# wzhe06/SparrowRecSys

Measured on AMD Instinct MI355X. Metric: ctr_samples_per_sec, higher is better.
Workload: dtype f32

## Files before the change

sparrowrecsys_amd/csrc/host_setup_v2.h:

```cpp
constexpr int V2_WAVES = 8;
struct V2Variant {
    int g_emb, kpc, h0c, h1c;
    size_t lds_bytes;
    void (*pack)(const V2Args, float*);
};
#define V2_LDS(G_EMB, DV, KPC, H0C, H1C, FOLD) \
    (sizeof(float) * (V2Lds<G_EMB, DV, KPC, H0C, H1C, FOLD>::total_pad + V2_WAVES * V2Lds<G_EMB, DV, KPC, H0C, H1C, FOLD>::stage_floats))
#define V2_VARIANT(G_EMB) {G_EMB, 1, 2, 1, V2_LDS(G_EMB, 4, 1, 2, 1, true), &k_v2_pack_image<G_EMB, 4, 1, 2, 1, true>}
const V2Variant kV2Variants[] = {
    V2_VARIANT(6),
    V2_VARIANT(4),
    V2_VARIANT(5), V2_VARIANT(3), V2_VARIANT(2),
};

struct V2JVariant {
    int g_big, njf, kpc;
    bool half;
    V2JKernel fn;
    V2JManyKernel fn_many;
};
#define V2J_VARIANT(G_BIG, NJF, HALF) \
    {G_BIG, NJF, 1, HALF, &k_deepfm_v2_joint<G_BIG, NJF, 1, 2, 1, V2_WAVES, HALF>, &k_deepfm_v2_joint_many<G_BIG, NJF, 1, 2, 1, V2_WAVES, HALF>}
#define V2J_BOTH(G_BIG, NJF) V2J_VARIANT(G_BIG, NJF, true), V2J_VARIANT(G_BIG, NJF, false)
const V2JVariant kV2JVariants[] = {
    V2J_BOTH(3, 3),
    V2J_BOTH(2, 2),
    V2J_BOTH(3, 2), V2J_BOTH(3, 1), V2J_BOTH(2, 3), V2J_BOTH(2, 1), V2J_BOTH(1, 3), V2J_BOTH(1, 2), V2J_BOTH(1, 1),
};

struct V2J1Variant { int g_big, njf; V2JKernel fn[2]; int image_floats; };
#define V2J1_VARIANT(G_BIG, NJF) \
    {G_BIG, NJF, {&k_deepfm_v2_joint1<G_BIG, NJF, false>, &k_deepfm_v2_joint1<G_BIG, NJF, true>}, V2J1Lds<G_BIG>::total_pad}
const V2J1Variant kV2J1Variants[] = {
    V2J1_VARIANT(3, 3), V2J1_VARIANT(2, 2), V2J1_VARIANT(3, 2), V2J1_VARIANT(3, 1), V2J1_VARIANT(2, 3), V2J1_VARIANT(2, 1),
    V2J1_VARIANT(1, 3), V2J1_VARIANT(1, 2), V2J1_VARIANT(1, 1),
};

bool match_v2_chain(sprk_engine* h) {
    const sprk_plan& p = h->plan;
    if (p.model_kind != SPRK_MODEL_DEEPFM_V2 || p.din.enabled || p.n_bufs != 2) return false;
    V2Args a;
    memset(&a, 0, sizeof(a));
    int g_emb = 0;
    while (g_emb < p.n_segs && p.segs[g_emb].kind == SPRK_SEG_ROWS) ++g_emb;
    if (g_emb < 1 || g_emb > V2_MAX_FIELDS) return false;
    if (p.n_id_cols > 8 || p.n_dense > 8 || p.n_dense < 1) return false;
    const int Dp = p.segs[0].row_stride;
    bool raw_over_4g = false;
    for (int g = 0; g < g_emb; ++g) {
        const sprk_seg& s = p.segs[g];
        if (s.row_stride != Dp || s.count * 4 != Dp || s.dst != g * Dp) return false;
        const size_t need = ((size_t)s.vocab + 1) * Dp * sizeof(float);
        if (h->slot_bytes[s.slot] < need) return false;
        if (need >= ((size_t)1 << 32)) raw_over_4g = true;
        a.emb_col[g] = s.field; a.emb_vocab[g] = s.vocab; a.table[g] = (const float*)h->slot_ptr[s.slot];
    }
    int si = g_emb;
    if (si >= p.n_segs || p.segs[si].kind != SPRK_SEG_DENSE || p.segs[si].field != 0 || p.segs[si].count > 8) return false;
    const int n_num = p.segs[si].count, num_off = p.segs[si].dst;
    ++si;
    if (si < p.n_segs && p.segs[si].kind == SPRK_SEG_ZERO) ++si;
// ... 62 lines not shown
        const V2Variant& vv = kV2Variants[v];
        if (!want_fold) continue;
        if (vv.g_emb == g_emb && vv.kpc == kpc && vv.h0c == h0c && vv.h1c == h1c) {
            V2Run run;
            memset(&run, 0, sizeof(run));
            size_t fo_floats = 0;
            for (int g = 0; g < g_emb; ++g) {
                int hit = -1;
                for (int i = 0; i < n_fo; ++i)
                    if (a.fo_col[i] == a.emb_col[g] && a.fo_vocab[i] == a.emb_vocab[g]) hit = i;
                if (hit < 0) return false;
                run.col[g] = a.emb_col[g]; run.vocab[g] = a.emb_vocab[g];
                run.table[g] = a.table[g];
                run.fo_off[g] = (unsigned)fo_floats;
                fo_floats += (size_t)a.emb_vocab[g] + 1;
            }
            if (fo_floats >= ((size_t)1 << 31)) return false;
            for (int g = 0; g < g_emb; ++g) {
                h->v2_w1_grp[g] = nullptr;
                for (int i = 0; i < n_fo; ++i)
                    if (a.fo_col[i] == a.emb_col[g] && a.fo_vocab[i] == a.emb_vocab[g]) h->v2_w1_grp[g] = a.w1[i];
            }
            run.F = a.F; run.ND = a.ND; run.n_num = a.n_num;
            run.h0w = a.h0w; run.fo_bias = a.fo_bias; run.head_bias = a.head_bias;
            h->v2run = run;
            h->v2 = a;
            h->v2_fo_floats = fo_floats;
            h->v2_variant = (int)v;
            h->rows_g_emb = g_emb;
            h->v2_rows_ok = kpc >= 1 && kpc <= 4 && h0c >= 1 && h1c >= 1 && !raw_over_4g;
            return true;
        }
    }
    if (kpc >= 1 && kpc <= 4 && h0c >= 1 && h1c >= 1 && !raw_over_4g) {
        h->v2 = a;
        h->rows_g_emb = g_emb;
        h->rows_from_v2 = true;
    }
    return false;
}

int setup_v2_joint(sprk_engine* h) {
    const V2Variant& vv = kV2Variants[h->v2_variant];
    if (vv.kpc != 1 || vv.h0c != 2 || vv.h1c != 1 || !h->tune.v2_joint) return SPRK_OK;
    const int KP = 16, H0 = 32, G = vv.g_emb;
    int big[V2_MAX_FIELDS], nbig = 0, jf[V2_MAX_FIELDS], njf = 0;
    for (int g = 0; g < G; ++g) {
        const long long v1 = (long long)h->v2run.vocab[g] + 1;
        if (v1 <= 32 && njf < V2J_MAX_JF) jf[njf++] = g;
        else big[nbig++] = g;
    }
    if (njf < 1 || nbig < 1 || nbig > 3) return SPRK_OK;
    bool half = h->tune.v2_half;
    float p_scale = 1.f, w_scale = 1.f;
    if (half) {
        std::vector<AbsmaxJob> rows_jobs;
        for (int b = 0; b < nbig; ++b) {
            const long long rows = (long long)h->v2run.vocab[big[b]] + 1;
            rows_jobs.push_back({h->v2_folded + (size_t)h->v2run.rowbase[big[b]] * (KP + 16), rows, KP + 16, KP, absmax_grid(rows * KP, 8192), 0});
        }
        SPRK_TRY(static_scale(rows_jobs, &p_scale));
        if (p_scale != 0.f) SPRK_TRY(static_scale({{h->v2.W0, (long long)H0, (G + 1) * KP, (G + 1) * KP, 8, 0}}, &w_scale));
        if (p_scale == 0.f || w_scale == 0.f) { half = false; p_scale = w_scale = 1.f; }
    }
    int variant = -1;
    for (size_t v = 0; v < sizeof(kV2JVariants) / sizeof(kV2JVariants[0]); ++v)
        if (kV2JVariants[v].g_big == nbig && kV2JVariants[v].njf == njf && kV2JVariants[v].half == half) variant = (int)v;
    if (variant < 0) return SPRK_OK;
    V2JRun& r = h->v2j_run;
    memset(&r, 0, sizeof(r));
    r.F = h->v2run.F; r.ND = h->v2run.ND; r.n_num = h->v2run.n_num;
    r.h0w = h->v2run.h0w; r.fo_bias = h->v2run.fo_bias; r.head_bias = h->v2run.head_bias;
    for (int b = 0; b < nbig; ++b) {
        r.big_col[b] = h->v2run.col[big[b]]; r.big_vocab[b] = h->v2run.vocab[big[b]];
        r.big_rowbase[b] = h->v2run.rowbase[big[b]]; r.big_grp[b] = big[b];
    }
    size_t small_floats = 0;
    for (int f = 0; f < njf; ++f) {
        r.j_col[f] = h->v2run.col[jf[f]]; r.j_vocab[f] = h->v2run.vocab[jf[f]];
        r.s_off[f] = (int)small_floats;
        small_floats += ((size_t)r.j_vocab[f] + 1) * V2J_SS;
    }
    small_floats = (small_floats + 255) & ~(size_t)255;
    r.wf_off = (int)small_floats;
    if (half) small_floats += ((size_t)H0 * 8 + 255) & ~(size_t)255;
    HIP_TRY(hipMalloc((void**)&h->v2j_tab, small_floats * sizeof(float)));
    HIP_TRY(hipMemset(h->v2j_tab, 0, small_floats * sizeof(float)));
    for (int f = 0; f < njf; ++f) {
        const int rows = r.j_vocab[f] + 1;
        hipLaunchKernelGGL(k_v2_fold_small, dim3((rows + 3) / 4), dim3(256), 0, 0,
                           h->v2_folded + (size_t)h->v2run.rowbase[jf[f]] * (KP + 16), KP, H0, jf[f], h->v2.W0, (G + 1) * KP,
                           h->v2.b0, f == 0 ? 1 : 0, h->v2j_tab + r.s_off[f], rows);
    }
    if (half)
        hipLaunchKernelGGL(k_v2j_fold_num, dim3(8), dim3(256), 0, 0, h->v2.W0, (G + 1) * KP, G * KP, h->v2.Wp[G], h->v2.ldp_num,
                           h->v2.bp[G], h->v2.n_num, KP, H0, h->v2j_tab + r.wf_off, h->v2j_tab + r.s_off[0], r.j_vocab[0] + 1);
    HIP_TRY(hipGetLastError());
    HIP_TRY(hipDeviceSynchronize());
    r.small_floats = (int)small_floats;
    r.tab0 = h->v2_folded;
    r.small = h->v2j_tab;
    r.w_scale = w_scale; r.unscale_h = 1.f / (p_scale * w_scale); r.unscale_s = 1.f / p_scale;
    if (half) {
        size_t big_rows = 0;
        for (int b = 0; b < nbig; ++b) big_rows += (size_t)r.big_vocab[b] + 1;
        if (big_rows * (KP + 16) * sizeof(float) >= ((size_t)1 << 32)) return fail(SPRK_EINVAL, "split rows exceed 32-bit offsets");
        SPRK_TRY(table_alloc(h, &h->v2j_big, big_rows * (KP + 16) * sizeof(float)));
        h->derived_bytes += big_rows * (KP + 16) * sizeof(float);
        size_t base = 0;
        for (int b = 0; b < nbig; ++b) {
            const long long rows = (long long)r.big_vocab[b] + 1;
            long long nb = (rows * 8 + 255) / 256;
            if (nb > 65536) nb = 65536;
            hipLaunchKernelGGL(k_v2_split_rows, dim3((unsigned)nb), dim3(256), 0, 0,
                               h->v2_folded + (size_t)r.big_rowbase[b] * (KP + 16), h->v2j_big + base * (KP + 16), rows, p_scale);
            r.big_rowbase[b] = (unsigned)base;
            base += (size_t)rows;
        }
        HIP_TRY(hipGetLastError());
        HIP_TRY(hipDeviceSynchronize());
        r.tab0 = h->v2j_big;
    }
    h->v2j_lds_bytes = vv.lds_bytes + small_floats * sizeof(float);
    SPRK_TRY(set_max_lds(kV2JVariants[variant].fn, h->v2j_lds_bytes));
    SPRK_TRY(set_max_lds(kV2JVariants[variant].fn_many, h->v2j_lds_bytes));
    h->v2j_variant = variant;
    if (half && h->tune.v2j_one) {
        for (size_t v = 0; v < sizeof(kV2J1Variants) / sizeof(kV2J1Variants[0]); ++v) {
            const V2J1Variant& ov = kV2J1Variants[v];
            if (ov.g_big != nbig || ov.njf != njf) continue;
            SPRK_TRY(dev_alloc(h, &h->v2j1_image, (size_t)ov.image_floats * sizeof(float)));
            hipLaunchKernelGGL(k_v2j1_pack_image, dim3(1), dim3(256), 0, 0, h->v2, r, nbig, G + 1, h->v2j1_image);
            HIP_TRY(hipGetLastError());
            HIP_TRY(hipDeviceSynchronize());
            const bool hoist = h->tune.v2j1_hoist >= 0 ? h->tune.v2j1_hoist != 0 : h->derived_bytes > ((size_t)256 << 20);
            h->v2j1_kernel = ov.fn[hoist];
            h->v2j1_waves = V2J1_WAVES_OF(hoist, nbig);
            h->v2j1_lds_bytes = ((size_t)ov.image_floats + small_floats + (size_t)h->v2j1_waves * 256) * sizeof(float);
            SPRK_TRY(set_max_lds(h->v2j1_kernel, h->v2j1_lds_bytes));
        }
    }
    return SPRK_OK;
}

int setup_v2_fold(sprk_engine* h) {
    const V2Variant& vv = kV2Variants[h->v2_variant];
    const int KP = vv.kpc * 16;
    h->v2_grid_cap = h->num_cus;
    SPRK_TRY(dev_alloc(h, &h->v2_fo_all, h->v2_fo_floats * sizeof(float)));
    for (int g = 0; g < vv.g_emb; ++g)
        HIP_TRY(hipMemcpy(h->v2_fo_all + h->v2run.fo_off[g], h->v2_w1_grp[g], ((size_t)h->v2run.vocab[g] + 1) * sizeof(float), hipMemcpyDeviceToDevice));
    h->v2run.fo_all = h->v2_fo_all;
    size_t rows_total = 0;
    for (int g = 0; g < vv.g_emb; ++g) { h->v2run.rowbase[g] = (unsigned)rows_total; rows_total += (size_t)h->v2run.vocab[g] + 1; }
    SPRK_TRY(table_alloc(h, &h->v2_folded, rows_total * (KP + 16) * sizeof(float)));
    for (int g = 0; g < vv.g_emb; ++g) {
        const long long rows = (long long)h->v2run.vocab[g] + 1;
        long long blocks = (rows + 3) / 4;
        if (blocks > 65536) blocks = 65536;
        hipLaunchKernelGGL(k_v2_fold, dim3((unsigned)blocks), dim3(256), 0, 0, h->v2.table[g], h->v2.ldp_emb,
                           h->v2.Wp[g], h->v2.ldp_emb, h->v2.bp[g], h->v2_w1_grp[g], h->v2.hfm, h->v2.n_hfm, h->v2.h0w,
                           h->v2_folded + (size_t)h->v2run.rowbase[g] * (KP + 16), KP, rows);
        HIP_TRY(hipGetLastError());
    }
    h->v2run.tab0 = h->v2_folded;
    HIP_TRY(hipDeviceSynchronize());
    SPRK_TRY(setup_v2_joint(h));
    if (h->v2j_variant < 0) {
        dev_free(h, h->v2_fo_all); h->v2_fo_all = nullptr;
        dev_free(h, h->v2_folded); h->v2_folded = nullptr;
        h->v2_variant = -1;
        h->rows_from_v2 = h->v2_rows_ok;
        return SPRK_OK;
    }
    h->derived_bytes += rows_total * (KP + 16) * sizeof(float);
    SPRK_TRY(dev_alloc(h, &h->v2_image, vv.lds_bytes));
    HIP_TRY(hipMemset(h->v2_image, 0, vv.lds_bytes));
    hipLaunchKernelGGL(vv.pack, dim3(1), dim3(256), 0, 0, h->v2, h->v2_image);
    HIP_TRY(hipGetLastError());
    HIP_TRY(hipDeviceSynchronize());
    return SPRK_OK;
}
```

sparrowrecsys_amd/csrc/k_chain_v2j.h:

```cpp

#define V2J_MAX_BIG 4
#define V2J_MAX_JF 3
#define V2J_SS 52

struct V2JRun {
    int F, ND, n_num;
    int big_col[V2J_MAX_BIG];
    int big_vocab[V2J_MAX_BIG];
    unsigned big_rowbase[V2J_MAX_BIG];
    int big_grp[V2J_MAX_BIG];
    int j_col[V2J_MAX_JF];
    int j_vocab[V2J_MAX_JF];
    int s_off[V2J_MAX_JF];
    int small_floats;
    int wf_off;
    const float* tab0;
    const float* small;
    float h0w, fo_bias, head_bias;
    int flags;
    float w_scale, unscale_h, unscale_s;
};

#define V2J_MB 64
struct V2JMany {
    const int* ids[V2J_MB];
    const float* dense[V2J_MB];
    float* out[V2J_MB];
    int n;
    int ntpb;
};

__device__ __forceinline__ void split_half4(f32x4 w, float scale, f16x4& hi, f16x4& lo) {
#pragma unroll
    for (int j = 0; j < 4; ++j) {
        const float x = w[j] * scale;
        const _Float16 h = (_Float16)x;
        hi[j] = h;
        lo[j] = (_Float16)(x - (float)h);
    }
}

static __global__ __launch_bounds__(256) void k_v2_absmax(const float* __restrict__ rows, long long nrows, int row_floats,
                                                   int ncols, unsigned* __restrict__ out) {
    float m = 0.f;
    const long long total = nrows * ncols;
    for (long long i = (long long)blockIdx.x * 256 + threadIdx.x; i < total; i += (long long)gridDim.x * 256) {
        const long long v = i / ncols;
        const int c = (int)(i - v * ncols);
        const float a = fabsf(rows[v * row_floats + c]);
        m = (a > m || a != a) ? a : m;
    }
    for (int d = 32; d >= 1; d >>= 1) { const float o = __shfl_xor(m, d); m = (o > m || o != o) ? o : m; }
    if ((threadIdx.x & 63) == 0) atomicMax(out, __float_as_uint(m));
}
static __global__ __launch_bounds__(256) void k_v2_count_small(const float* __restrict__ rows, long long nrows, int row_floats, int ncols,
                                                        float thresh, unsigned long long* __restrict__ out) {
    unsigned small = 0, nz = 0;
    const long long total = nrows * ncols;
    for (long long i = (long long)blockIdx.x * 256 + threadIdx.x; i < total; i += (long long)gridDim.x * 256) {
        const long long v = i / ncols;
        const int c = (int)(i - v * ncols);
        const float a = fabsf(rows[v * row_floats + c]);
        nz += a > 0.f;
        small += (a > 0.f && a < thresh);
    }
    for (int d = 32; d >= 1; d >>= 1) { small += __shfl_xor(small, d); nz += __shfl_xor(nz, d); }
    if ((threadIdx.x & 63) == 0) { atomicAdd(out, (unsigned long long)small); atomicAdd(out + 1, (unsigned long long)nz); }
}
static __global__ __launch_bounds__(256) void k_v2_split_rows(const float* __restrict__ src, float* __restrict__ dst,
                                                       long long nrows, float scale) {
    const long long total = nrows * 8;
    for (long long i = (long long)blockIdx.x * 256 + threadIdx.x; i < total; i += (long long)gridDim.x * 256) {
        const long long v = i >> 3;
// ... 11 lines not shown
}

static __global__ __launch_bounds__(256) void k_v2_fold_small(const float* __restrict__ folded, int KP, int H0, int grp,
                                                       const float* __restrict__ W0, int ldw0,
                                                       const float* __restrict__ b0, int add_b0,
                                                       float* __restrict__ out, int rows) {
    const int FS = KP + 16;
    for (int v = blockIdx.x * 4 + (threadIdx.x >> 6); v < rows; v += gridDim.x * 4) {
        const int col = threadIdx.x & 63;
        const float* prow = folded + (size_t)v * FS;
        float acc = 0.f;
        if (col < KP) {
            acc = prow[col];
        } else if (col < KP + H0) {
            const int m = col - KP;
            acc = add_b0 ? b0[m] : 0.f;
            const float* w = W0 + (size_t)m * ldw0 + grp * KP;
            for (int k = 0; k < KP; ++k) acc = fmaf(w[k], prow[k], acc);
        } else if (col == KP + H0) {
            acc = prow[KP];
        }
        if (col < V2J_SS) out[(size_t)v * V2J_SS + col] = acc;
    }
}

static __global__ __launch_bounds__(256) void k_v2j_fold_num(const float* __restrict__ W0, int ldw0, int num_off,
                                                      const float* __restrict__ Wn, int ldn, const float* __restrict__ bn,
                                                      int n_num, int KP, int H0, float* __restrict__ wf,
                                                      float* __restrict__ rows0, int nrows0) {
    for (int i = blockIdx.x * 256 + threadIdx.x; i < H0 * 8; i += gridDim.x * 256) {
        const int m = i >> 3, k = i & 7;
        double acc = 0.0;
        if (k < n_num)
            for (int n = 0; n < KP; ++n) acc += (double)W0[(size_t)m * ldw0 + num_off + n] * (double)Wn[(size_t)n * ldn + k];
        wf[i] = (float)acc;
    }
    for (int i = blockIdx.x * 256 + threadIdx.x; i < nrows0 * H0; i += gridDim.x * 256) {
        const int v = i / H0, m = i - v * H0;
        double acc = 0.0;
        for (int n = 0; n < KP; ++n) acc += (double)W0[(size_t)m * ldw0 + num_off + n] * (double)bn[n];
        rows0[(size_t)v * V2J_SS + KP + m] = (float)((double)rows0[(size_t)v * V2J_SS + KP + m] + acc);
    }
}

__device__ __forceinline__ f32x4 fma4s(f32x4 a, float b, f32x4 c) {
    return f32x4{__builtin_fmaf(a.x, b, c.x), __builtin_fmaf(a.y, b, c.y), __builtin_fmaf(a.z, b, c.z), __builtin_fmaf(a.w, b, c.w)};
}
__device__ __forceinline__ float dot4f(f32x4 a, f32x4 b) {
    return __builtin_fmaf(a.w, b.w, __builtin_fmaf(a.z, b.z, __builtin_fmaf(a.y, b.y, a.x * b.x)));
}
__device__ __forceinline__ f32x4 sq_diff4(f32x4 s, f32x4 p) {
    return f32x4{__builtin_fmaf(s.x, s.x, -(p.x * p.x)), __builtin_fmaf(s.y, s.y, -(p.y * p.y)), __builtin_fmaf(s.z, s.z, -(p.z * p.z)),
                 __builtin_fmaf(s.w, s.w, -(p.w * p.w))};
}

template <int G_BIG, int NJF>
struct V2JSet {
    f32x4 x[G_BIG];
    int so[NJF];
    f32x4 xn;
    float w1a;
};

template <int G_BIG, int NJF, int KPC, int H0C, int H1C, int WAVES, bool HALF, bool MB>
__device__ __forceinline__ void v2j_body(const V2JRun& A, const int* __restrict__ ids, const float* __restrict__ dense,
                                         float* __restrict__ out, int B, int* __restrict__ err,
                                         const float* __restrict__ image, const V2JMany* __restrict__ Mp) {
    constexpr int G_EMB = G_BIG + NJF;
    using LD = V2Lds<G_EMB, 4, KPC, H0C, H1C, true>;
    using Set = V2JSet<G_BIG, NJF>;
    constexpr int KP = LD::KP, H0 = H0C * 16;
    constexpr unsigned RB = (KP + 16) * 4;
    static_assert(KP + H0 + 1 <= V2J_SS, "small-field row layout");
    constexpr int NKR = HALF ? 1 : (G_BIG + 1) * KPC;
    static_assert(KPC == 1, "row layout: one 16-float chunk of projections per field");
    static_assert(G_BIG >= 1 && G_BIG <= 3 && NJF >= 1 && NJF <= V2J_MAX_JF, "field split");
    const int tid = threadIdx.x;
    const int lane = tid & 63;
    const int wave = __builtin_amdgcn_readfirstlane(tid >> 6);
    const int r = lane & 15, q = lane >> 4;
    const f32x4 zero = f32x4{0.f, 0.f, 0.f, 0.f};
    const int m_ntpb = MB ? Mp->ntpb : 0;
    const int ntasks = MB ? Mp->n * m_ntpb : (B + 15) >> 4;
    const int task_stride = gridDim.x * WAVES;
    const int wave_global = blockIdx.x * WAVES + wave;
    auto batch_of = [&](int tk, int& tl) {
        if constexpr (MB) {
            const int b = __builtin_amdgcn_readfirstlane(tk / m_ntpb);
            tl = tk - b * m_ntpb;
            return b;
        } else {
            tl = tk;
            return 0;
        }
    };
    float* stage = smem + LD::total_pad + wave * LD::stage_floats;
    const float* small_s = smem + LD::total_pad + WAVES * LD::stage_floats;
    const float* wq = smem + 4 * q;
    bool bad = false;
    const bool aligned = !(A.flags & 1);
    auto clampt = [&](int tk) { return tk < ntasks ? tk : ntasks - 1; };
    const int* const ids0 = ids;
    const float* const dense0 = dense;

    auto ld_raw = [&](int tkg, f32x4& raw) {
        int tk;
// ... 18 lines not shown
            const bool isid = lane < 32;
            const int j = isid ? lane : lane - 32;
            const int n4 = 4 * (isid ? A.F : A.ND);
            if (j < n4) st4(stage + (isid ? 0 : 128) + 4 * j, raw);
        } else {
            stage_task_slow(stage, ids, dense, A.F, A.ND, tk, B, lane);
        }
        const int* sid_row = reinterpret_cast<const int*>(stage) + r * A.F;
        unsigned sid[G_BIG];
#pragma unroll
        for (int b = 0; b < G_BIG; ++b) {
            const int id = sid_row[A.big_col[b]];
            bad |= (unsigned)(id + 1) > (unsigned)A.big_vocab[b];
            sid[b] = min((unsigned)id, (unsigned)A.big_vocab[b]) + A.big_rowbase[b];
        }
#pragma unroll
        for (int f = 0; f < NJF; ++f) {
            const int id = sid_row[A.j_col[f]];
            bad |= (unsigned)(id + 1) > (unsigned)A.j_vocab[f];
            S.so[f] = A.s_off[f] + (int)min((unsigned)id, (unsigned)A.j_vocab[f]) * V2J_SS;
        }
        {
            const float* nrow = stage + 128 + r * A.ND;
            const int c0 = 4 * q, last = A.n_num - 1;
            if constexpr (HALF) {
                S.xn.x = nrow[min(q, last)];
                S.xn.y = nrow[min(q + 4, last)];
            } else {
                S.xn.x = nrow[min(c0 + 0, last)];
                S.xn.y = nrow[min(c0 + 1, last)];
                S.xn.z = nrow[min(c0 + 2, last)];
                S.xn.w = nrow[min(c0 + 3, last)];
            }
        }
        const char* tb = reinterpret_cast<const char*>(A.tab0);
#pragma unroll
        for (int b = 0; b < G_BIG; ++b) S.x[b] = *reinterpret_cast<const f32x4*>(tb + (sid[b] * RB + 16u * q));
        {
            unsigned s0 = sid[0] * RB, s1 = sid[G_BIG > 1 ? 1 : 0] * RB, s2 = sid[G_BIG > 2 ? 2 : 0] * RB;
            asm("" : "+v"(s0), "+v"(s1), "+v"(s2));
            unsigned so = s0;
            if (G_BIG > 1) so = q == 1 ? s1 : so;
            if (G_BIG > 2) so = q == 2 ? s2 : so;
            S.w1a = *reinterpret_cast<const float*>(tb + (so + 4u * KP));
        }
    };

    f32x4 rW0[H0C][NKR], rW1[H1C][H0C];
    f32x4 rwn[KPC], rbpn[KPC], rb1[H1C], rhfm[KPC], rhd[H1C];
    f32x4 rfn = zero;
    float rwn8[2] = {0.f, 0.f}, rfn8[2] = {0.f, 0.f}, rwf[H0C][2];
    f16x8 hWa[HALF ? G_BIG : 1][H0C], hWb[HALF ? G_BIG : 1][H0C];
    f16x8 hSel = {0, 0, 0, 0, 0, 0, 0, 0};
    auto load_weights = [&]() {
        const float* w0r = wq + LD::off_w0 + r * LD::S0;
#pragma unroll
        for (int n0 = 0; n0 < H0C; ++n0) {
            if constexpr (HALF) {
                rwf[n0][0] = small_s[A.wf_off + (n0 * 16 + r) * 8 + q];
                rwf[n0][1] = small_s[A.wf_off + (n0 * 16 + r) * 8 + q + 4];
            } else {
                rW0[n0][0] = ld4(w0r + n0 * 16 * LD::S0 + 16 * G_EMB);
            }
#pragma unroll
            for (int b = 0; b < G_BIG; ++b) {
                const f32x4 w = ld4(w0r + n0 * 16 * LD::S0 + 16 * A.big_grp[b]);
                if constexpr (HALF) {
                    f16x4 hi, lo;
                    split_half4(w, A.w_scale, hi, lo);
                    hWa[b][n0] = f16x8{hi[0], hi[1], hi[2], hi[3], hi[0], hi[1], hi[2], hi[3]};
                    hWb[b][n0] = f16x8{lo[0], lo[1], lo[2], lo[3], lo[0], lo[1], lo[2], lo[3]};
                } else {
                    rW0[n0][(HALF ? 0 : 1 + b)] = w;
                }
            }
        }
        if constexpr (HALF) {
#pragma unroll
            for (int e = 0; e < 8; ++e) hSel[e] = (4 * q + (e & 3) == r) ? (_Float16)1.0f : (_Float16)0.0f;
        }
#pragma unroll
        for (int n1 = 0; n1 < H1C; ++n1) {
#pragma unroll
            for (int j = 0; j < H0C; ++j) rW1[n1][j] = ld4(wq + LD::off_w1 + (n1 * 16 + r) * LD::S1 + 16 * j);
            rb1[n1] = ld4(wq + LD::off_b1 + n1 * 16);
            rhd[n1] = ld4(wq + LD::off_hd + n1 * 16);
        }
#pragma unroll
        for (int nb = 0; nb < KPC; ++nb) {
            rwn[nb] = ld4(wq + LD::off_wn + (nb * 16 + r) * LD::SN);
            rbpn[nb] = ld4(wq + LD::off_bp + G_EMB * KP + nb * 16);
            rhfm[nb] = ld4(wq + LD::off_hfm + nb * 16);
        }
        rfn = ld4(smem + LD::off_fn + 4 * (q & 1));
        if constexpr (HALF) {
            rwn8[0] = smem[LD::off_wn + r * LD::SN + q];
            rwn8[1] = smem[LD::off_wn + r * LD::SN + q + 4];
            rfn8[0] = smem[LD::off_fn + q];
            rfn8[1] = smem[LD::off_fn + q + 4];
        }
    };

    auto compute = [&](const Set& S) -> float {
#pragma clang fp contract(off)
        const f32x4 pnum = S.xn;
        f32x4 pn;
        if constexpr (HALF) {
            const f32x4 e = __builtin_amdgcn_mfma_f32_16x16x4f32(rwn8[0], pnum.x, rbpn[0], 0, 0, 0);
            const f32x4 o = __builtin_amdgcn_mfma_f32_16x16x4f32(rwn8[1], pnum.y, zero, 0, 0, 0);
            pn = e + o;
        } else {
            f32x4 e = rbpn[0], o = zero;
            e = __builtin_amdgcn_mfma_f32_16x16x4f32(rwn[0].x, pnum.x, e, 0, 0, 0);
            o = __builtin_amdgcn_mfma_f32_16x16x4f32(rwn[0].y, pnum.y, o, 0, 0, 0);
            e = __builtin_amdgcn_mfma_f32_16x16x4f32(rwn[0].z, pnum.z, e, 0, 0, 0);
            o = __builtin_amdgcn_mfma_f32_16x16x4f32(rwn[0].w, pnum.w, o, 0, 0, 0);
            pn = e + o;
        }
        float zz = ((q < G_BIG) ? S.w1a : 0.f) + (HALF ? __builtin_fmaf(rfn8[1], pnum.y, rfn8[0] * pnum.x) : ((q < 2) ? dot4f(rfn, pnum) : 0.f));
        f32x4 sp = ld4(small_s + S.so[0] + 4 * q), sq[H0C];
#pragma unroll
        for (int n0 = 0; n0 < H0C; ++n0) sq[n0] = ld4(small_s + S.so[0] + KP + 16 * n0 + 4 * q);
        float ssc = small_s[S.so[0] + KP + H0];
#pragma unroll
        for (int f = 1; f < NJF; ++f) {
            sp += ld4(small_s + S.so[f] + 4 * q);
#pragma unroll
            for (int n0 = 0; n0 < H0C; ++n0) sq[n0] += ld4(small_s + S.so[f] + KP + 16 * n0 + 4 * q);
            ssc += small_s[S.so[f] + KP + H0];
        }
        zz += (q == 3) ? ssc : 0.f;
        f32x4 hA[H0C], hB[H0C];
#pragma unroll
        for (int n0 = 0; n0 < H0C; ++n0) { hA[n0] = sq[n0]; hB[n0] = zero; }
        f32x4 s = sp + pn;
        if constexpr (HALF) {
            f32x4 aFa[H0C], aFb[H0C], aS = zero;
#pragma unroll
            for (int n0 = 0; n0 < H0C; ++n0) { aFa[n0] = zero; aFb[n0] = zero; }
            __builtin_amdgcn_sched_barrier(0);
#pragma unroll
            for (int b = 0; b < G_BIG; ++b) {
                const f16x8 xb = __builtin_bit_cast(f16x8, S.x[b]);
#pragma unroll
                for (int n0 = 0; n0 < H0C; ++n0) aFa[n0] = __builtin_amdgcn_mfma_f32_16x16x32_f16(hWa[b][n0], xb, aFa[n0], 0, 0, 0);
                aS = __builtin_amdgcn_mfma_f32_16x16x32_f16(hSel, xb, aS, 0, 0, 0);
#pragma unroll
                for (int n0 = 0; n0 < H0C; ++n0) aFb[n0] = __builtin_amdgcn_mfma_f32_16x16x32_f16(hWb[b][n0], xb, aFb[n0], 0, 0, 0);
                __builtin_amdgcn_sched_barrier(0);
            }
#pragma unroll
            for (int st = 0; st < 2; ++st)
#pragma unroll
                for (int n0 = 0; n0 < H0C; ++n0)
                    hA[n0] = __builtin_amdgcn_mfma_f32_16x16x4f32(rwf[n0][st], st ? pnum.y : pnum.x, hA[n0], 0, 0, 0);
            s = fma4s(aS, A.unscale_s, s);
#pragma unroll
            for (int n0 = 0; n0 < H0C; ++n0) hB[n0] = (aFa[n0] + aFb[n0]) * A.unscale_h;
        } else {
#pragma unroll
            for (int b = 0; b < G_BIG; ++b) s += S.x[b];
            __builtin_amdgcn_sched_barrier(0);
#pragma unroll
            for (int c = 0; c < NKR; c += 2) {
                const bool hb = c + 1 < NKR;
                const f32x4 pa = c == 0 ? pn : S.x[c > 0 ? c - 1 : 0];
                const f32x4 pb = !hb ? zero : S.x[hb ? c : 0];
#pragma unroll
                for (int st = 0; st < 4; ++st) {
#pragma unroll
                    for (int n0 = 0; n0 < H0C; ++n0)
                        hA[n0] = __builtin_amdgcn_mfma_f32_16x16x4f32(rW0[n0][c][st], pa[st], hA[n0], 0, 0, 0);
                    if (hb) {
#pragma unroll
                        for (int n0 = 0; n0 < H0C; ++n0)
                            hB[n0] = __builtin_amdgcn_mfma_f32_16x16x4f32(rW0[n0][hb ? c + 1 : c][st], pb[st], hB[n0], 0, 0, 0);
                    }
                    __builtin_amdgcn_sched_barrier(0);
                }
            }
        }
        f32x4 h0[H0C];
#pragma unroll
        for (int n0 = 0; n0 < H0C; ++n0) h0[n0] = relu4_fast(hA[n0] + hB[n0]);
        float z = dot4f(rhfm[0], sq_diff4(s, pn));
#pragma unroll
        for (int n1 = 0; n1 < H1C; ++n1) {
            f32x4 e = rb1[n1], o = zero;
#pragma unroll
            for (int j = 0; j < H0C; ++j) {
                e = __builtin_amdgcn_mfma_f32_16x16x4f32(rW1[n1][j].x, h0[j].x, e, 0, 0, 0);
                o = __builtin_amdgcn_mfma_f32_16x16x4f32(rW1[n1][j].y, h0[j].y, o, 0, 0, 0);
                e = __builtin_amdgcn_mfma_f32_16x16x4f32(rW1[n1][j].z, h0[j].z, e, 0, 0, 0);
                o = __builtin_amdgcn_mfma_f32_16x16x4f32(rW1[n1][j].w, h0[j].w, o, 0, 0, 0);
            }
            z += dot4f(rhd[n1], relu4_fast(e + o));
        }
        z += zz;
        z = rows4_sum(z);
        return sigmoidf_fast(z + A.h0w * A.fo_bias + A.head_bias);
    };
    auto store = [&](int tkg, float score) {
        int tk;
        const int bi = batch_of(tkg, tk);
        float* out_b = MB ? Mp->out[bi] : out;
        const int m = tk * 16 + r;
        if (q == 0 && m < B) out_b[m] = score;
    };

    Set SA, SB;
    f32x4 rawA = zero, rawB = zero;
    int tA = wave_global, tB = wave_global + task_stride;
    if (ntasks > 0) {
        ld_raw(clampt(tA), rawA);
        ld_raw(clampt(tB), rawB);
    }
#pragma unroll 1
    for (int c = wave; c < LD::total_pad / 256; c += WAVES) lds_dma16(image + c * 256 + lane * 4, smem + c * 256);
#pragma unroll 1
    for (int c = wave; c < A.small_floats / 256; c += WAVES) lds_dma16(A.small + c * 256 + lane * 4, smem + LD::total_pad + WAVES * LD::stage_floats + c * 256);
    const bool two = tA < ntasks && ntasks <= 2 * task_stride;
    constexpr int NG = G_BIG + 1;
    static_assert(NG < 16, "s_waitcnt immediate below encodes vmcnt < 16");
    if (two) {
        gather(tA, rawA, SA);
        __builtin_amdgcn_s_waitcnt(0x0F70 | NG);
    } else {
        __builtin_amdgcn_s_waitcnt(0x0F70);
    }
    __builtin_amdgcn_s_barrier();
    load_weights();
    if (tA >= ntasks) {
    } else if (two) {
        gather(clampt(tB), rawB, SB);
        store(tA, compute(SA));
        if (tB < ntasks) store(tB, compute(SB));
    } else {
        gather(tA, rawA, SA);
        ld_raw(clampt(tA + 2 * task_stride), rawA);
        gather(clampt(tB), rawB, SB);
        ld_raw(clampt(tB + 2 * task_stride), rawB);
        for (;;) {
            store(tA, compute(SA));
            tA += 2 * task_stride;
            gather(clampt(tA), rawA, SA);
            ld_raw(clampt(tA + 2 * task_stride), rawA);
            if (tB >= ntasks) break;
            store(tB, compute(SB));
            tB += 2 * task_stride;
// ... 20 lines not shown
```

sparrowrecsys_amd/csrc/k_chain_v2j1.h:

```cpp

#define V2J1_WAVES 16
#define V2J1_WAVES_HOIST 8
#define V2J1_WAVES_OF(HOIST, G_BIG) (((HOIST) && (G_BIG) >= 3) ? V2J1_WAVES_HOIST : V2J1_WAVES)
#define V2J1_MAX_TASKS 16384

template <int G_BIG>
struct V2J1Lds {
    static constexpr int off_frag = 0;
    static constexpr int S1 = 36;
    static constexpr int off_w1 = off_frag + G_BIG * 2 * 256;
    static constexpr int off_b1 = off_w1 + 16 * S1;
    static constexpr int off_hd = off_b1 + 16;
    static constexpr int off_bpn = off_hd + 16;
    static constexpr int off_hfm = off_bpn + 16;
    static constexpr int off_wn8 = off_hfm + 16;
    static constexpr int off_fn8 = off_wn8 + 128;
    static constexpr int total = off_fn8 + 8;
    static constexpr int total_pad = (total + 255) & ~255;
};

static __global__ __launch_bounds__(256) void k_v2j1_pack_image(const V2Args A, const V2JRun R, int g_big, int G, float* __restrict__ img) {
    const int tid = threadIdx.x;
    const int off_w1 = g_big * 2 * 256, off_b1 = off_w1 + 16 * 36, off_hd = off_b1 + 16, off_bpn = off_hd + 16,
              off_hfm = off_bpn + 16, off_wn8 = off_hfm + 16, off_fn8 = off_wn8 + 128, total_pad = (off_fn8 + 8 + 255) & ~255;
    for (int i = tid; i < total_pad; i += 256) img[i] = 0.f;
    __syncthreads();
    f16x8* frag = reinterpret_cast<f16x8*>(img);
    for (int i = tid; i < g_big * 2 * 64; i += 256) {
        const int l = i & 63, n0 = (i >> 6) & 1, b = i >> 7, r = l & 15, q = l >> 4;
        const f32x4 w = ld4(A.W0 + (size_t)(n0 * 16 + r) * (G * 16) + 16 * R.big_grp[b] + 4 * q);
        f16x4 hi, lo;
        split_half4(w, R.w_scale, hi, lo);
        frag[(b * 2 + n0) * 64 + l] = f16x8{hi[0], hi[1], hi[2], hi[3], lo[0], lo[1], lo[2], lo[3]};
    }
    for (int i = tid; i < 16 * 32; i += 256) img[off_w1 + (i >> 5) * 36 + (i & 31)] = A.W1[i];
    if (tid < 16) {
        img[off_b1 + tid] = A.b1[tid];
        img[off_hd + tid] = tid < A.n_hdeep ? A.hdeep[tid] : 0.f;
        img[off_bpn + tid] = A.bp[G - 1][tid];
        img[off_hfm + tid] = tid < A.n_hfm ? A.hfm[tid] : 0.f;
    }
    if (tid < 128) img[off_wn8 + tid] = (tid & 7) < A.n_num ? A.Wp[G - 1][(size_t)(tid >> 3) * A.ldp_num + (tid & 7)] : 0.f;
    if (tid < 8) img[off_fn8 + tid] = tid < A.n_num ? A.h0w * A.fo_num_w[tid] : 0.f;
}

template <int G_BIG, int NJF, bool HOIST = false>
__global__ __launch_bounds__(V2J1_WAVES_OF(HOIST, G_BIG) * 64, 4) void k_deepfm_v2_joint1(const V2JRun A, const int* __restrict__ ids,
                                                                       const float* __restrict__ dense, float* __restrict__ out, int B,
                                                                       int* __restrict__ err, const float* __restrict__ image) {
#pragma clang fp contract(off)
    using LD = V2J1Lds<G_BIG>;
    constexpr int WAVES = V2J1_WAVES_OF(HOIST, G_BIG), KP = 16, H0C = 2;
    constexpr unsigned RB = (KP + 16) * 4;
    static_assert(G_BIG >= 1 && G_BIG <= 3 && NJF >= 1 && NJF <= V2J_MAX_JF, "field split");
    const int tid = threadIdx.x;
    const int lane = tid & 63;
    const int wave = __builtin_amdgcn_readfirstlane(tid >> 6);
    const int r = lane & 15, q = lane >> 4;
    const f32x4 zero = f32x4{0.f, 0.f, 0.f, 0.f};
    const int ntasks = (B + 15) >> 4;
    const int tk = blockIdx.x * WAVES + wave;
    const bool work = tk < ntasks;
    const float* small_s = smem + LD::total_pad;
    float* stage = smem + LD::total_pad + A.small_floats + wave * 256;
    const bool fast = work && !(A.flags & 1) && tk * 16 + 16 <= B;

    f32x4 raw = zero;
    if (fast) {
        const bool isid = lane < 32;
        const int j = isid ? lane : lane - 32;
        const int n4 = 4 * (isid ? A.F : A.ND);
        const float* src = isid ? reinterpret_cast<const float*>(ids) + (size_t)tk * 16 * A.F : dense + (size_t)tk * 16 * A.ND;
        raw = ld4(src + 4 * (j < n4 ? j : 0));
    }
#pragma unroll 1
    for (int c = wave; c < LD::total_pad / 256; c += WAVES) lds_dma16(image + c * 256 + lane * 4, smem + c * 256);
#pragma unroll 1
    for (int c = wave; c < A.small_floats / 256; c += WAVES) lds_dma16(A.small + c * 256 + lane * 4, smem + LD::total_pad + c * 256);

    __builtin_amdgcn_s_waitcnt(0x0F70);
    __builtin_amdgcn_s_barrier();
    if (!work) return;
    f16x8 wa[G_BIG][H0C], wb[G_BIG][H0C], hSel;
    f16x8 wt[G_BIG][H0C];
    auto read_frags = [&]() {
        const f16x8* frag = reinterpret_cast<const f16x8*>(smem + LD::off_frag) + lane;
#pragma unroll
        for (int b = 0; b < G_BIG; ++b)
#pragma unroll
            for (int n0 = 0; n0 < H0C; ++n0) wt[b][n0] = frag[(b * 2 + n0) * 64];
    };
    auto expand_frags = [&]() {
#pragma unroll
        for (int b = 0; b < G_BIG; ++b)
#pragma unroll
            for (int n0 = 0; n0 < H0C; ++n0) {
                const f16x8 t = wt[b][n0];
                wa[b][n0] = f16x8{t[0], t[1], t[2], t[3], t[0], t[1], t[2], t[3]};
                wb[b][n0] = f16x8{t[4], t[5], t[6], t[7], t[4], t[5], t[6], t[7]};
            }
        const int d = r - 4 * q;
        const unsigned lo01 = d == 0 ? 0x00003C00u : d == 1 ? 0x3C000000u : 0u, lo23 = d == 2 ? 0x00003C00u : d == 3 ? 0x3C000000u : 0u;
        typedef unsigned u32x4 __attribute__((ext_vector_type(4)));
        hSel = __builtin_bit_cast(f16x8, u32x4{lo01, lo23, lo01, lo23});
    };
    if constexpr (HOIST) {
        read_frags();
        expand_frags();
        __builtin_amdgcn_sched_barrier(0);
    }
    f32x4 x[G_BIG];
    int so[NJF];
    float xn0 = 0.f, xn1 = 0.f, w1a = 0.f;
    bool bad = false;
#pragma unroll
    for (int b = 0; b < G_BIG; ++b) x[b] = zero;
#pragma unroll
    for (int f = 0; f < NJF; ++f) so[f] = 0;
    {
        if (fast) {
            const bool isid = lane < 32;
            const int j = isid ? lane : lane - 32;
            const int n4 = 4 * (isid ? A.F : A.ND);
            if (j < n4) st4(stage + (isid ? 0 : 128) + 4 * j, raw);
        } else {
            stage_task_slow(stage, ids, dense, A.F, A.ND, tk, B, lane);
        }
        const int* sid_row = reinterpret_cast<const int*>(stage) + r * A.F;
        unsigned sid[G_BIG];
#pragma unroll
        for (int b = 0; b < G_BIG; ++b) {
            const int id = sid_row[A.big_col[b]];
            bad |= (unsigned)(id + 1) > (unsigned)A.big_vocab[b];
            sid[b] = min((unsigned)id, (unsigned)A.big_vocab[b]) + A.big_rowbase[b];
        }
#pragma unroll
        for (int f = 0; f < NJF; ++f) {
            const int id = sid_row[A.j_col[f]];
            bad |= (unsigned)(id + 1) > (unsigned)A.j_vocab[f];
            so[f] = A.s_off[f] + (int)min((unsigned)id, (unsigned)A.j_vocab[f]) * V2J_SS;
        }
        {
            const float* nrow = stage + 128 + r * A.ND;
            const int last = A.n_num - 1;
            xn0 = nrow[min(q, last)];
            xn1 = nrow[min(q + 4, last)];
        }
        const char* tb = reinterpret_cast<const char*>(A.tab0);
#pragma unroll
        for (int b = 0; b < G_BIG; ++b) x[b] = *reinterpret_cast<const f32x4*>(tb + (sid[b] * RB + 16u * q));
        {
            unsigned s0 = sid[0] * RB, s1 = sid[G_BIG > 1 ? 1 : 0] * RB, s2 = sid[G_BIG > 2 ? 2 : 0] * RB;
            asm("" : "+v"(s0), "+v"(s1), "+v"(s2));
            unsigned sx = s0;
            if (G_BIG > 1) sx = q == 1 ? s1 : sx;
            if (G_BIG > 2) sx = q == 2 ? s2 : sx;
            w1a = *reinterpret_cast<const float*>(tb + (sx + 4u * KP));
        }
    }

    const float* vq = smem + 4 * q;
    const f32x4 rbpn = ld4(vq + LD::off_bpn);
    const float rwn8a = smem[LD::off_wn8 + r * 8 + q], rwn8b = smem[LD::off_wn8 + r * 8 + q + 4];
    const float rfn8a = smem[LD::off_fn8 + q], rfn8b = smem[LD::off_fn8 + q + 4];
    f32x4 sp = ld4(small_s + so[0] + 4 * q), sq[H0C];
#pragma unroll
    for (int n0 = 0; n0 < H0C; ++n0) sq[n0] = ld4(small_s + so[0] + KP + 16 * n0 + 4 * q);
    float ssc = small_s[so[0] + KP + 32];
#pragma unroll
    for (int f = 1; f < NJF; ++f) {
        sp += ld4(small_s + so[f] + 4 * q);
#pragma unroll
        for (int n0 = 0; n0 < H0C; ++n0) sq[n0] += ld4(small_s + so[f] + KP + 16 * n0 + 4 * q);
        ssc += small_s[so[f] + KP + 32];
    }
    if constexpr (!HOIST) { read_frags(); expand_frags(); }
    float rwf[H0C][2];
    {
        const float* wf = small_s + A.wf_off + r * 8 + q;
#pragma unroll
        for (int n0 = 0; n0 < H0C; ++n0) { rwf[n0][0] = wf[n0 * 128]; rwf[n0][1] = wf[n0 * 128 + 4]; }
    }
    f32x4 rW1[H0C];
#pragma unroll
    for (int j = 0; j < H0C; ++j) rW1[j] = ld4(vq + LD::off_w1 + r * LD::S1 + 16 * j);
    const f32x4 rb1 = ld4(vq + LD::off_b1), rhd = ld4(vq + LD::off_hd), rhfm = ld4(vq + LD::off_hfm);
    f32x4 pn;
    {
        const f32x4 e = __builtin_amdgcn_mfma_f32_16x16x4f32(rwn8a, xn0, rbpn, 0, 0, 0);
        const f32x4 o = __builtin_amdgcn_mfma_f32_16x16x4f32(rwn8b, xn1, zero, 0, 0, 0);
        pn = e + o;
    }
    const float zz_num = __builtin_fmaf(rfn8b, xn1, rfn8a * xn0);
    float zz = 0.f;
    if constexpr (HOIST) {
        zz = ((q < G_BIG) ? w1a : 0.f) + zz_num;
        zz += (q == 3) ? ssc : 0.f;
    }
    f32x4 hA[H0C], hB[H0C];
#pragma unroll
    for (int n0 = 0; n0 < H0C; ++n0) hA[n0] = sq[n0];
#pragma unroll
    for (int st = 0; st < 2; ++st)
#pragma unroll
        for (int n0 = 0; n0 < H0C; ++n0) hA[n0] = __builtin_amdgcn_mfma_f32_16x16x4f32(rwf[n0][st], st ? xn1 : xn0, hA[n0], 0, 0, 0);
    f32x4 s = sp + pn;
    __builtin_amdgcn_sched_barrier(0);
    {
        f32x4 aFa[H0C], aFb[H0C], aS = zero;
#pragma unroll
        for (int n0 = 0; n0 < H0C; ++n0) { aFa[n0] = zero; aFb[n0] = zero; }
#pragma unroll
        for (int b = 0; b < G_BIG; ++b) {
            const f16x8 xb = __builtin_bit_cast(f16x8, x[b]);
#pragma unroll
            for (int n0 = 0; n0 < H0C; ++n0) aFa[n0] = __builtin_amdgcn_mfma_f32_16x16x32_f16(wa[b][n0], xb, aFa[n0], 0, 0, 0);
            aS = __builtin_amdgcn_mfma_f32_16x16x32_f16(hSel, xb, aS, 0, 0, 0);
#pragma unroll
            for (int n0 = 0; n0 < H0C; ++n0) aFb[n0] = __builtin_amdgcn_mfma_f32_16x16x32_f16(wb[b][n0], xb, aFb[n0], 0, 0, 0);
            __builtin_amdgcn_sched_barrier(0);
        }
        s = fma4s(aS, A.unscale_s, s);
#pragma unroll
        for (int n0 = 0; n0 < H0C; ++n0) hB[n0] = (aFa[n0] + aFb[n0]) * A.unscale_h;
    }
    f32x4 h0[H0C];
#pragma unroll
    for (int n0 = 0; n0 < H0C; ++n0) h0[n0] = relu4_fast(hA[n0] + hB[n0]);
    float z = dot4f(rhfm, sq_diff4(s, pn));
    {
        f32x4 e = rb1, o = zero;
#pragma unroll
        for (int j = 0; j < H0C; ++j) {
            e = __builtin_amdgcn_mfma_f32_16x16x4f32(rW1[j].x, h0[j].x, e, 0, 0, 0);
            o = __builtin_amdgcn_mfma_f32_16x16x4f32(rW1[j].y, h0[j].y, o, 0, 0, 0);
            e = __builtin_amdgcn_mfma_f32_16x16x4f32(rW1[j].z, h0[j].z, e, 0, 0, 0);
            o = __builtin_amdgcn_mfma_f32_16x16x4f32(rW1[j].w, h0[j].w, o, 0, 0, 0);
        }
        z += dot4f(rhd, relu4_fast(e + o));
    }
    if constexpr (!HOIST) {
        zz = ((q < G_BIG) ? w1a : 0.f) + zz_num;
        zz += (q == 3) ? ssc : 0.f;
    }
    z += zz;
    z = rows4_sum(z);
    const float score = sigmoidf_fast(z + A.h0w * A.fo_bias + A.head_bias);
    const int m = tk * 16 + r;
    if (q == 0 && m < B) out[m] = score;
    if (__ballot(bad) != 0 && lane == 0) atomicOr(err, 1);
}
```

sparrowrecsys_amd/csrc/tu_kernels.h:

```cpp
#include <hip/hip_runtime.h>
#include <dlfcn.h>
#include <unistd.h>

#include <cstdarg>
#include <cstdint>
#include <cstdio>
#include <cstdlib>
#include <cstring>
#include <new>
#include <string>
#include <type_traits>
#include <thread>
#include <vector>

#include "sparrow_hip.h"

#include "host_common.h"
#include "k_tile_forward.h"
#include "k_chain_v2.h"
#include "k_chain_v2j.h"
#include "k_chain_v2j1.h"
#include "k_rows_chain.h"
#include "k_din_attn.h"
#include "dyn_split.h"
#include "k_din_cols.h"
#include "k_din_tail.h"
#include "k_din_fused.h"
#include "k_chain_v1.h"
#include "k_mlp_rows.h"
#include "k_emb_rank.h"
#include "k_emb_topk.h"
#include "k_als_topk.h"
#include "k_dien_seq.h"
#include "k_dien_mfma.h"
#include "k_dien_fused.h"
#include "k_peer_gather.h"
#include "k_csv_pack.h"
#include "k_pack_columns.h"
#include "k_feature_join.h"
#include "k_rank_scores.h"
#include "k_operators.h"
#include "tu_instances.h"
```

Measured before the change: 17.09 billion.

## Run deep layer-1 matmul as split-f16 MFMA with dynamic activation scaling

In the half-precision DeepFM joint kernels, the second MLP layer (32->16) was eight f32 16x16x4 MFMAs per row tile; it now uses three f16 16x16x32 MFMAs on hi/lo split operands. The W1 weights are prepacked into f16 hi/lo fragments in the LDS image using a static scale, and activations get a per-tile dynamic scale from a row max. This is meant to cut MFMA issue count and the f32 W1 register/LDS footprint, in exchange for a row-max reduction and split/convert work per tile, plus some accuracy risk from the f16 split.

After: 17.10 billion (median of 3 runs). No clear change (+0.1%).

```diff
diff --git a/sparrowrecsys_amd/csrc/host_setup_v2.h b/sparrowrecsys_amd/csrc/host_setup_v2.h
--- a/sparrowrecsys_amd/csrc/host_setup_v2.h
+++ b/sparrowrecsys_amd/csrc/host_setup_v2.h
@@ -2,11 +2,12 @@
 struct V2Variant {
     int g_emb, kpc, h0c, h1c;
     size_t lds_bytes;
+    int off_w1;
     void (*pack)(const V2Args, float*);
 };
 #define V2_LDS(G_EMB, DV, KPC, H0C, H1C, FOLD) \
     (sizeof(float) * (V2Lds<G_EMB, DV, KPC, H0C, H1C, FOLD>::total_pad + V2_WAVES * V2Lds<G_EMB, DV, KPC, H0C, H1C, FOLD>::stage_floats))
-#define V2_VARIANT(G_EMB) {G_EMB, 1, 2, 1, V2_LDS(G_EMB, 4, 1, 2, 1, true), &k_v2_pack_image<G_EMB, 4, 1, 2, 1, true>}
+#define V2_VARIANT(G_EMB) {G_EMB, 1, 2, 1, V2_LDS(G_EMB, 4, 1, 2, 1, true), V2Lds<G_EMB, 4, 1, 2, 1, true>::off_w1, &k_v2_pack_image<G_EMB, 4, 1, 2, 1, true>}
 const V2Variant kV2Variants[] = {
     V2_VARIANT(6),
     V2_VARIANT(4),
@@ -175,7 +176,7 @@
     }
     if (njf < 1 || nbig < 1 || nbig > 3) return SPRK_OK;
     bool half = h->tune.v2_half;
-    float p_scale = 1.f, w_scale = 1.f;
+    float p_scale = 1.f, w_scale = 1.f, w1_scale = 1.f;
     if (half) {
         std::vector<AbsmaxJob> rows_jobs;
         for (int b = 0; b < nbig; ++b) {
@@ -184,7 +185,10 @@
         }
         SPRK_TRY(static_scale(rows_jobs, &p_scale));
         if (p_scale != 0.f) SPRK_TRY(static_scale({{h->v2.W0, (long long)H0, (G + 1) * KP, (G + 1) * KP, 8, 0}}, &w_scale));
-        if (p_scale == 0.f || w_scale == 0.f) { half = false; p_scale = w_scale = 1.f; }
+        float mx1 = 0.f;
+        if (p_scale != 0.f && w_scale != 0.f) SPRK_TRY(static_scale({{h->v2.W1, 16, H0, H0, 8, 0}}, &w1_scale, &mx1));
+        if (!(mx1 > 0.f)) w1_scale = 0.f;
+        if (p_scale == 0.f || w_scale == 0.f || w1_scale == 0.f) { half = false; p_scale = w_scale = w1_scale = 1.f; }
     }
     int variant = -1;
     for (size_t v = 0; v < sizeof(kV2JVariants) / sizeof(kV2JVariants[0]); ++v)
@@ -224,6 +228,7 @@
     r.tab0 = h->v2_folded;
     r.small = h->v2j_tab;
     r.w_scale = w_scale; r.unscale_h = 1.f / (p_scale * w_scale); r.unscale_s = 1.f / p_scale;
+    r.unscale_1 = 1.f / w1_scale;
     if (half) {
         size_t big_rows = 0;
         for (int b = 0; b < nbig; ++b) big_rows += (size_t)r.big_vocab[b] + 1;
@@ -254,6 +259,8 @@
             if (ov.g_big != nbig || ov.njf != njf) continue;
             SPRK_TRY(dev_alloc(h, &h->v2j1_image, (size_t)ov.image_floats * sizeof(float)));
             hipLaunchKernelGGL(k_v2j1_pack_image, dim3(1), dim3(256), 0, 0, h->v2, r, nbig, G + 1, h->v2j1_image);
+            hipLaunchKernelGGL(k_dyn_pack_w, dim3(4), dim3(256), 0, 0, h->v2.W1, H0, 16, H0, w1_scale,
+                               reinterpret_cast<_Float16*>(h->v2j1_image + nbig * 2 * 256), H0);
             HIP_TRY(hipGetLastError());
             HIP_TRY(hipDeviceSynchronize());
             const bool hoist = h->tune.v2j1_hoist >= 0 ? h->tune.v2j1_hoist != 0 : h->derived_bytes > ((size_t)256 << 20);
@@ -300,6 +307,10 @@
     SPRK_TRY(dev_alloc(h, &h->v2_image, vv.lds_bytes));
     HIP_TRY(hipMemset(h->v2_image, 0, vv.lds_bytes));
     hipLaunchKernelGGL(vv.pack, dim3(1), dim3(256), 0, 0, h->v2, h->v2_image);
+    static_assert(V2Lds<6, 4, 1, 2, 1, true>::S1 * 16 >= 2 * 256, "deep1's fragments fit where its f32 rows were");
+    if (kV2JVariants[h->v2j_variant].half)
+        hipLaunchKernelGGL(k_dyn_pack_w, dim3(4), dim3(256), 0, 0, h->v2.W1, 32, 16, 32, 1.f / h->v2j_run.unscale_1,
+                           reinterpret_cast<_Float16*>(h->v2_image + vv.off_w1), 32);
     HIP_TRY(hipGetLastError());
     HIP_TRY(hipDeviceSynchronize());
     return SPRK_OK;
diff --git a/sparrowrecsys_amd/csrc/k_chain_v2j.h b/sparrowrecsys_amd/csrc/k_chain_v2j.h
--- a/sparrowrecsys_amd/csrc/k_chain_v2j.h
+++ b/sparrowrecsys_amd/csrc/k_chain_v2j.h
@@ -19,6 +19,7 @@
     float h0w, fo_bias, head_bias;
     int flags;
     float w_scale, unscale_h, unscale_s;
+    float unscale_1;
 };
 
 #define V2J_MB 64
@@ -136,6 +137,19 @@
 __device__ __forceinline__ f32x4 sq_diff4(f32x4 s, f32x4 p) {
     return f32x4{__builtin_fmaf(s.x, s.x, -(p.x * p.x)), __builtin_fmaf(s.y, s.y, -(p.y * p.y)), __builtin_fmaf(s.z, s.z, -(p.z * p.z)),
                  __builtin_fmaf(s.w, s.w, -(p.w * p.w))};
+}
+
+__device__ __forceinline__ f32x4 v2j_deep1_split(f32x4 h0a, f32x4 h0b, f16x8 w1h, f16x8 w1l, float unscale_1, f32x4 b1) {
+    float mx = fmaxf(fmaxf(fmaxf(h0a.x, h0a.y), fmaxf(h0a.z, h0a.w)), fmaxf(fmaxf(h0b.x, h0b.y), fmaxf(h0b.z, h0b.w)));
+    mx = rows4_max(mx);
+    float scale, inv;
+    dyn_scale(mx, unscale_1, scale, inv);
+    f16x8 bh, bl;
+    dyn_split8(h0a, h0b, scale, bh, bl);
+    f32x4 acc = __builtin_amdgcn_mfma_f32_16x16x32_f16(w1l, bh, f32x4{0.f, 0.f, 0.f, 0.f}, 0, 0, 0);
+    acc = __builtin_amdgcn_mfma_f32_16x16x32_f16(w1h, bl, acc, 0, 0, 0);
+    acc = __builtin_amdgcn_mfma_f32_16x16x32_f16(w1h, bh, acc, 0, 0, 0);
+    return fma4s(acc, lone_scalar(inv), b1);
 }
 
 template <int G_BIG, int NJF>
@@ -260,6 +274,8 @@
     float rwn8[2] = {0.f, 0.f}, rfn8[2] = {0.f, 0.f}, rwf[H0C][2];
     f16x8 hWa[HALF ? G_BIG : 1][H0C], hWb[HALF ? G_BIG : 1][H0C];
     f16x8 hSel = {0, 0, 0, 0, 0, 0, 0, 0};
+    f16x8 hW1h[H1C], hW1l[H1C];
+    static_assert(!HALF || H0C == 2, "HALF: deep1's input is one K = 32 block");
     auto load_weights = [&]() {
         const float* w0r = wq + LD::off_w0 + r * LD::S0;
 #pragma unroll
@@ -289,8 +305,13 @@
         }
 #pragma unroll
         for (int n1 = 0; n1 < H1C; ++n1) {
-#pragma unroll
-            for (int j = 0; j < H0C; ++j) rW1[n1][j] = ld4(wq + LD::off_w1 + (n1 * 16 + r) * LD::S1 + 16 * j);
+            if constexpr (HALF) {
+                hW1h[n1] = __builtin_bit_cast(f16x8, ld4(smem + LD::off_w1 + (n1 * 2 + 0) * 256 + lane * 4));
+                hW1l[n1] = __builtin_bit_cast(f16x8, ld4(smem + LD::off_w1 + (n1 * 2 + 1) * 256 + lane * 4));
+            } else {
+#pragma unroll
+                for (int j = 0; j < H0C; ++j) rW1[n1][j] = ld4(wq + LD::off_w1 + (n1 * 16 + r) * LD::S1 + 16 * j);
+            }
             rb1[n1] = ld4(wq + LD::off_b1 + n1 * 16);
             rhd[n1] = ld4(wq + LD::off_hd + n1 * 16);
         }
@@ -394,15 +415,19 @@
         float z = dot4f(rhfm[0], sq_diff4(s, pn));
 #pragma unroll
         for (int n1 = 0; n1 < H1C; ++n1) {
-            f32x4 e = rb1[n1], o = zero;
-#pragma unroll
-            for (int j = 0; j < H0C; ++j) {
-                e = __builtin_amdgcn_mfma_f32_16x16x4f32(rW1[n1][j].x, h0[j].x, e, 0, 0, 0);
-                o = __builtin_amdgcn_mfma_f32_16x16x4f32(rW1[n1][j].y, h0[j].y, o, 0, 0, 0);
-                e = __builtin_amdgcn_mfma_f32_16x16x4f32(rW1[n1][j].z, h0[j].z, e, 0, 0, 0);
-                o = __builtin_amdgcn_mfma_f32_16x16x4f32(rW1[n1][j].w, h0[j].w, o, 0, 0, 0);
-            }
-            z += dot4f(rhd[n1], relu4_fast(e + o));
+            if constexpr (HALF) {
+                z += dot4f(rhd[n1], relu4_fast(v2j_deep1_split(h0[0], h0[H0C - 1], hW1h[n1], hW1l[n1], A.unscale_1, rb1[n1])));
+            } else {
+                f32x4 e = rb1[n1], o = zero;
+#pragma unroll
+                for (int j = 0; j < H0C; ++j) {
+                    e = __builtin_amdgcn_mfma_f32_16x16x4f32(rW1[n1][j].x, h0[j].x, e, 0, 0, 0);
+                    o = __builtin_amdgcn_mfma_f32_16x16x4f32(rW1[n1][j].y, h0[j].y, o, 0, 0, 0);
+                    e = __builtin_amdgcn_mfma_f32_16x16x4f32(rW1[n1][j].z, h0[j].z, e, 0, 0, 0);
+                    o = __builtin_amdgcn_mfma_f32_16x16x4f32(rW1[n1][j].w, h0[j].w, o, 0, 0, 0);
+                }
+                z += dot4f(rhd[n1], relu4_fast(e + o));
+            }
         }
         z += zz;
         z = rows4_sum(z);
diff --git a/sparrowrecsys_amd/csrc/k_chain_v2j1.h b/sparrowrecsys_amd/csrc/k_chain_v2j1.h
--- a/sparrowrecsys_amd/csrc/k_chain_v2j1.h
+++ b/sparrowrecsys_amd/csrc/k_chain_v2j1.h
@@ -7,9 +7,8 @@
 template <int G_BIG>
 struct V2J1Lds {
     static constexpr int off_frag = 0;
-    static constexpr int S1 = 36;
     static constexpr int off_w1 = off_frag + G_BIG * 2 * 256;
-    static constexpr int off_b1 = off_w1 + 16 * S1;
+    static constexpr int off_b1 = off_w1 + 2 * 256;
     static constexpr int off_hd = off_b1 + 16;
     static constexpr int off_bpn = off_hd + 16;
     static constexpr int off_hfm = off_bpn + 16;
@@ -21,7 +20,7 @@
 
 static __global__ __launch_bounds__(256) void k_v2j1_pack_image(const V2Args A, const V2JRun R, int g_big, int G, float* __restrict__ img) {
     const int tid = threadIdx.x;
-    const int off_w1 = g_big * 2 * 256, off_b1 = off_w1 + 16 * 36, off_hd = off_b1 + 16, off_bpn = off_hd + 16,
+    const int off_w1 = g_big * 2 * 256, off_b1 = off_w1 + 2 * 256, off_hd = off_b1 + 16, off_bpn = off_hd + 16,
               off_hfm = off_bpn + 16, off_wn8 = off_hfm + 16, off_fn8 = off_wn8 + 128, total_pad = (off_fn8 + 8 + 255) & ~255;
     for (int i = tid; i < total_pad; i += 256) img[i] = 0.f;
     __syncthreads();
@@ -33,7 +32,6 @@
         split_half4(w, R.w_scale, hi, lo);
         frag[(b * 2 + n0) * 64 + l] = f16x8{hi[0], hi[1], hi[2], hi[3], lo[0], lo[1], lo[2], lo[3]};
     }
-    for (int i = tid; i < 16 * 32; i += 256) img[off_w1 + (i >> 5) * 36 + (i & 31)] = A.W1[i];
     if (tid < 16) {
         img[off_b1 + tid] = A.b1[tid];
         img[off_hd + tid] = tid < A.n_hdeep ? A.hdeep[tid] : 0.f;
@@ -104,8 +102,14 @@
         typedef unsigned u32x4 __attribute__((ext_vector_type(4)));
         hSel = __builtin_bit_cast(f16x8, u32x4{lo01, lo23, lo01, lo23});
     };
+    f16x8 w1h, w1l;
+    auto read_w1 = [&]() {
+        w1h = __builtin_bit_cast(f16x8, ld4(smem + LD::off_w1 + lane * 4));
+        w1l = __builtin_bit_cast(f16x8, ld4(smem + LD::off_w1 + 256 + lane * 4));
+    };
     if constexpr (HOIST) {
         read_frags();
+        read_w1();
         expand_frags();
         __builtin_amdgcn_sched_barrier(0);
     }
@@ -181,9 +185,7 @@
 #pragma unroll
         for (int n0 = 0; n0 < H0C; ++n0) { rwf[n0][0] = wf[n0 * 128]; rwf[n0][1] = wf[n0 * 128 + 4]; }
     }
-    f32x4 rW1[H0C];
-#pragma unroll
-    for (int j = 0; j < H0C; ++j) rW1[j] = ld4(vq + LD::off_w1 + r * LD::S1 + 16 * j);
+    if constexpr (!HOIST) read_w1();
     const f32x4 rb1 = ld4(vq + LD::off_b1), rhd = ld4(vq + LD::off_hd), rhfm = ld4(vq + LD::off_hfm);
     f32x4 pn;
     {
@@ -228,17 +230,7 @@
 #pragma unroll
     for (int n0 = 0; n0 < H0C; ++n0) h0[n0] = relu4_fast(hA[n0] + hB[n0]);
     float z = dot4f(rhfm, sq_diff4(s, pn));
-    {
-        f32x4 e = rb1, o = zero;
-#pragma unroll
-        for (int j = 0; j < H0C; ++j) {
-            e = __builtin_amdgcn_mfma_f32_16x16x4f32(rW1[j].x, h0[j].x, e, 0, 0, 0);
-            o = __builtin_amdgcn_mfma_f32_16x16x4f32(rW1[j].y, h0[j].y, o, 0, 0, 0);
-            e = __builtin_amdgcn_mfma_f32_16x16x4f32(rW1[j].z, h0[j].z, e, 0, 0, 0);
-            o = __builtin_amdgcn_mfma_f32_16x16x4f32(rW1[j].w, h0[j].w, o, 0, 0, 0);
-        }
-        z += dot4f(rhd, relu4_fast(e + o));
-    }
+    z += dot4f(rhd, relu4_fast(v2j_deep1_split(h0[0], h0[1], w1h, w1l, A.unscale_1, rb1)));
     if constexpr (!HOIST) {
         zz = ((q < G_BIG) ? w1a : 0.f) + zz_num;
         zz += (q == 3) ? ssc : 0.f;
diff --git a/sparrowrecsys_amd/csrc/tu_kernels.h b/sparrowrecsys_amd/csrc/tu_kernels.h
--- a/sparrowrecsys_amd/csrc/tu_kernels.h
+++ b/sparrowrecsys_amd/csrc/tu_kernels.h
@@ -17,12 +17,12 @@
 
 #include "host_common.h"
 #include "k_tile_forward.h"
+#include "dyn_split.h"
 #include "k_chain_v2.h"
 #include "k_chain_v2j.h"
 #include "k_chain_v2j1.h"
 #include "k_rows_chain.h"
 #include "k_din_attn.h"
-#include "dyn_split.h"
 #include "k_din_cols.h"
 #include "k_din_tail.h"
 #include "k_din_fused.h"
```
